# aleph-zero-foundation/sha2-on-cq-halo2

Hardware: AMD Instinct MI355X
Metric: sha256_cq_create_proof_k18: MSM Mscalar/s over proof-generation wall-clock (ms_per_step) (higher is better)
Workload: dtype u256-montgomery

## Files before the change

sha2_on_cq_halo2_amd/csrc/capi.hip:

```cpp
#include "ctx.hpp"
#include "comm.hpp"
#include "msm.hpp"
#include "poly.hpp"
#include <cstring>

using namespace cq;

const NttTables* cq_ctx::tables_for(uint32_t log_n, const Fr& omega, int* rc) {
  for (auto& t : ntt_cache)
    if (t->log_n == log_n && t->omega == omega) return t.get();
  if (ntt_cache.size() >= 16) {
    hipStreamSynchronize(stream);
    ntt_cache.erase(ntt_cache.begin());
  }
  auto t = std::make_unique<NttTables>();
  if (t->build(log_n, omega, stream) != 0) {
    *rc = fail(CQ_ERR_HIP, "building NTT twiddle tables failed");
    return nullptr;
  }
  ntt_cache.push_back(std::move(t));
  return ntt_cache.back().get();
}

extern "C" {

const char* cq_version(void) { return "cq_halo2_amd 0.1 (gfx950)"; }

int cq_ctx_create(int device, void* hip_stream, cq_ctx** out) {
  if (!out) return CQ_ERR_ARG;
  int count = 0;
  if (hipGetDeviceCount(&count) != hipSuccess || count <= 0 || device < 0 || device >= count)
    return CQ_ERR_NO_DEVICE;
  if (hipSetDevice(device) != hipSuccess) return CQ_ERR_HIP;
  cq_ctx* c = new cq_ctx();
  c->device = device;
  if (hip_stream) {
    c->stream = (hipStream_t)hip_stream;
  } else {
    if (hipStreamCreateWithFlags(&c->stream, hipStreamNonBlocking) != hipSuccess) {
      delete c;
      return CQ_ERR_HIP;
    }
    c->own_stream = true;
  }
  *out = c;
  return CQ_OK;
}

void cq_ctx_destroy(cq_ctx* c) {
  if (!c) return;
  hipSetDevice(c->device);
  for (cq_ctx* lane : c->lanes) cq_ctx_destroy(lane);
  c->lanes.clear();
  hipStreamSynchronize(c->stream);
  if (c->aux_stream) hipStreamSynchronize(c->aux_stream);
  c->ntt_cache.clear();
  cq::comm_rccl_destroy(c);
  for (const cq::GrowBuf& b : c->scratch)
    if (b.ptr) hipFree(b.ptr);
  for (const cq::GrowBuf* b : {&c->pinned, &c->pinned_msm, &c->pinned_small, &c->pinned_comm})
    if (b->ptr) hipHostFree(b->ptr);
  if (c->comm_event) hipEventDestroy(c->comm_event);
  for (auto& g : c->graphs) hipGraphExecDestroy(g.exec);
  if (c->prof_entries) hipHostFree(c->prof_entries);
  if (c->copy_done) hipEventDestroy(c->copy_done);
  if (c->copy_stream) hipStreamDestroy(c->copy_stream);
  if (c->msm_tail_event) hipEventDestroy(c->msm_tail_event);
  if (c->aux_done) hipEventDestroy(c->aux_done);
  if (c->aux_stream) hipStreamDestroy(c->aux_stream);
  if (c->fb_table) hipFree(c->fb_table);
  for (auto& t : c->msm_tables) hipFree(t.table);
  if (c->own_stream) hipStreamDestroy(c->stream);
  delete c;
}

const char* cq_last_error(const cq_ctx* c) { return c ? c->err.c_str() : "null context"; }

int cq_rccl_unique_id(uint8_t id[CQ_RCCL_UNIQUE_ID_BYTES]) {
  if (!id) return CQ_ERR_ARG;
  return cq::comm_rccl_unique_id(id);
}
int cq_ctx_comm_init_rccl(cq_ctx* c, uint32_t rank, uint32_t world, const uint8_t id[CQ_RCCL_UNIQUE_ID_BYTES]) {
  if (!c || !id || world == 0 || rank >= world) return CQ_ERR_ARG;
  CQ_HIP(c, hipSetDevice(c->device));
  return cq::comm_rccl_init(c, rank, world, id);
}
int cq_ctx_comm_selftest(cq_ctx* c) {
  if (!c) return CQ_ERR_ARG;
  CQ_HIP(c, hipSetDevice(c->device));
  return cq::comm_rccl_selftest(c);
}
int cq_ctx_comm_destroy(cq_ctx* c) {
  if (!c) return CQ_ERR_ARG;
  cq::comm_rccl_destroy(c);
  return CQ_OK;
}

int cq_ctx_set_hip_graphs(cq_ctx* c, int on) {
  if (!c) return CQ_ERR_ARG;
  c->graphs_on = on ? 1 : 0;
  return CQ_OK;
}

int cq_ctx_sync(cq_ctx* c) {
  if (!c) return CQ_ERR_ARG;
  CQ_HIP(c, hipStreamSynchronize(c->stream));
  return CQ_OK;
}

void* cq_ctx_stream(cq_ctx* c) { return c ? (void*)c->stream : nullptr; }

int cq_dev_alloc(cq_ctx* c, size_t bytes, void** dptr) {
  if (!c || !dptr) return CQ_ERR_ARG;
  CQ_HIP(c, hipSetDevice(c->device));
  CQ_HIP(c, hipMalloc(dptr, bytes ? bytes : 1));
  return CQ_OK;
}
int cq_dev_free(cq_ctx* c, void* dptr) {
  if (!c) return CQ_ERR_ARG;
  if (!dptr) return CQ_OK;
  CQ_HIP(c, hipStreamSynchronize(c->stream));
  msm_unregister_tables(c, dptr);
  CQ_HIP(c, hipFree(dptr));
  return CQ_OK;
}
int cq_dev_upload(cq_ctx* c, void* dst, const void* src, size_t bytes) {
  if (!c || (!dst && bytes) || (!src && bytes)) return CQ_ERR_ARG;
  if (!bytes) return CQ_OK;
  CQ_HIP(c, hipMemcpyAsync(dst, src, bytes, hipMemcpyHostToDevice, c->stream));
  CQ_HIP(c, hipStreamSynchronize(c->stream));
  return CQ_OK;
}
int cq_dev_download(cq_ctx* c, void* dst, const void* src, size_t bytes) {
  if (!c || (!dst && bytes) || (!src && bytes)) return CQ_ERR_ARG;
  if (!bytes) return CQ_OK;
  CQ_HIP(c, hipMemcpyAsync(dst, src, bytes, hipMemcpyDeviceToHost, c->stream));
  CQ_HIP(c, hipStreamSynchronize(c->stream));
  return CQ_OK;
}
int cq_dev_memset(cq_ctx* c, void* dptr, int value, size_t bytes) {
  if (!c || (!dptr && bytes)) return CQ_ERR_ARG;
  if (!bytes) return CQ_OK;
  CQ_HIP(c, hipMemsetAsync(dptr, value, bytes, c->stream));
  return CQ_OK;
}

int cq_profile_enable(cq_ctx* c, int on) {
  if (!c) return CQ_ERR_ARG;
  if (on && !c->prof_entries) {
    hipError_t e = hipHostMalloc((void**)&c->prof_entries, cq_ctx::PROF_COUNTERS * sizeof(uint32_t), hipHostMallocDefault);
    if (e != hipSuccess) return c->hip_fail(e, "hipHostMalloc(profile counters)");
  }
  c->prof_on = on != 0;
  return CQ_OK;
}

int cq_profile_read(cq_ctx* c, int id, double* total_ms, uint64_t* calls) {
  if (!c || !total_ms || !calls) return CQ_ERR_ARG;
  CQ_HIP(c, hipStreamSynchronize(c->stream));
  double tot = 0;
  uint64_t n = 0;
  if (id == CQ_PROF_MSM_ENTRIES) {
    for (size_t i = 0; i < c->prof_entries_n; i++) n += c->prof_entries[i];
    c->prof_entries_n = 0;
    *total_ms = 0;
    *calls = n;
    return CQ_OK;
  }
  std::vector<cq_ctx::ProfSpan> keep;
  for (auto& sp : c->prof_spans) {
    if (sp.id != id) {
      keep.push_back(sp);
      continue;
    }
    float ms = 0;
    if (hipEventElapsedTime(&ms, sp.a, sp.b) == hipSuccess) {
      tot += ms;
      n++;
    }
    hipEventDestroy(sp.a);
    hipEventDestroy(sp.b);
  }
  c->prof_spans.swap(keep);
  *total_ms = tot;
  *calls = n;
  return CQ_OK;
}

static int fft_dev(cq_ctx* c, const Fr* in, Fr* out, uint32_t log_n, const Fr& omega) {
  return domain_fft(c, in, out, log_n, omega, 1, (size_t)1 << log_n, (size_t)1 << log_n);
}

int cq_best_fft_dev(cq_ctx* c, const uint64_t* in_dev, uint64_t* out_dev, uint32_t log_n,
                    const uint64_t omega[4]) {
  if (!c || !in_dev || !out_dev || !omega || log_n > FR_S) return CQ_ERR_ARG;
  CQ_HIP(c, hipSetDevice(c->device));
  return fft_dev(c, (const Fr*)in_dev, (Fr*)out_dev, log_n, Fr::from_limbs64(omega));
}

int cq_best_fft(cq_ctx* c, uint64_t* a, uint32_t log_n, const uint64_t omega[4]) {
  if (!c || !a || !omega || log_n > FR_S) return CQ_ERR_ARG;
  CQ_HIP(c, hipSetDevice(c->device));
  const size_t bytes = ((size_t)1 << log_n) * sizeof(Fr);
  void *din, *dout;
  int rc;
  if ((rc = c->ensure_scratch(Scratch::EntryA, bytes, &din)) != CQ_OK) return rc;
  if ((rc = c->ensure_scratch(Scratch::EntryB, bytes, &dout)) != CQ_OK) return rc;
  CQ_HIP(c, hipMemcpyAsync(din, a, bytes, hipMemcpyHostToDevice, c->stream));
  if ((rc = fft_dev(c, (const Fr*)din, (Fr*)dout, log_n, Fr::from_limbs64(omega))) != CQ_OK) return rc;
  CQ_HIP(c, hipMemcpyAsync(a, dout, bytes, hipMemcpyDeviceToHost, c->stream));
  CQ_HIP(c, hipStreamSynchronize(c->stream));
  return CQ_OK;
}

}
```

sha2_on_cq_halo2_amd/csrc/capi_msm.hip:

```cpp
#include <algorithm>
#include <cstdlib>
#include <cstring>
#include <string>
#include <vector>
#include "ctx.hpp"
#include "msm.hpp"
#include "g1fft.hpp"
#include "setup.hpp"
#include "cq.hpp"
#include "serde.hpp"
#include "msm_g2.hpp"

using namespace cq;

uint32_t msm_table_window_bits(size_t n) {
  if (const char* e = getenv("CQ_TABLE_C")) {
    const long v = atol(e);
    if (v >= (long)MSM_TABLE_C_MIN && v <= (long)MSM_TABLE_C_MAX) return (uint32_t)v;
  }
  return n >= ((size_t)1 << 20) ? 17u : MSM_TABLE_C;
}

static uint32_t pick_c(cq_ctx* c, uint32_t n) {
  if (c->msm_c) return c->msm_c;
  return msm_window_bits(n);
}

int msm_multi_begin(cq_ctx* c, const Fr* const* scalars, const G1Affine* const* bases, const size_t* lens, size_t count,
                    MsmPending& pend) {
  pend.launches.clear();
  pend.count = count;
  for (size_t j = 0; j < count; j++)
    if (lens[j] > 0x7fffffffull) return c->fail(CQ_ERR_ARG, "msm: len too large");
  uint32_t want_c = 0;
  {
    size_t longest = 0;
    for (size_t j = 0; j < count; j++)
      if (lens[j] > longest)
        if (const cq_ctx::MsmTable* t = c->find_msm_table(bases[j], lens[j])) { longest = lens[j]; want_c = t->c; }
  }
  size_t done = 0, slots = 0;
  while (done < count) {
    MsmPending::Launch ln;
    ln.first = done;
    if (lens[done] == 0) {
      ln.batch = 1;
      ln.empty = true;
      pend.launches.push_back(ln);
      done++;
      continue;
    }
    const cq_ctx::MsmTable* t0 = c->find_msm_table(bases[done], lens[done], nullptr, want_c);
    const bool pre = t0 != nullptr;
    uint32_t nmax = (uint32_t)lens[done];
    uint32_t batch = 1;
    while (done + batch < count && batch < MSM_MAX_BATCH) {
      const size_t l = lens[done + batch];
      if (l == 0) break;
      const cq_ctx::MsmTable* t = c->find_msm_table(bases[done + batch], l, nullptr, want_c);
      if ((t != nullptr) != pre) break;
      if (pre && t->c != t0->c) break;
      if (!pre && l != lens[done]) break;
      nmax = std::max(nmax, (uint32_t)l);
      batch++;
    }
    ln.short_path = !pre && !c->msm_c && nmax <= MSM_SHORT_MAX;
    const uint32_t cb = pre ? t0->c : ln.short_path ? MSM_SHORT_C : pick_c(c, nmax);
    while (batch > 1 && MsmLayout(nmax, cb, batch, pre).total > ((size_t)32 << 30)) batch = (batch + 1) / 2;
    ln.batch = batch;
    ln.pre = pre;
    ln.c = cb;
    ln.nmax = nmax;
    MsmLayout L(nmax, cb, batch, pre);
    ln.W = L.W;
    ln.Wb = L.Wb;
    ln.M = L.M;
    ln.cols = L.cols;
    ln.slot = slots;
    slots += (size_t)MSM_SET_POINTS * batch * L.Wb;
    pend.launches.push_back(ln);
    done += batch;
  }
  void *wsums = nullptr, *host = nullptr;
  int rc;
  if (slots) {
    if ((rc = c->ensure_scratch(Scratch::MsmSums, slots * sizeof(G1Jac), &wsums)) != CQ_OK) return rc;
    if ((rc = c->ensure_pinned_msm(slots * sizeof(G1Jac), &host)) != CQ_OK) return rc;
  }
  pend.host = host;
  pend.slots = slots;
  for (auto& ln : pend.launches) {
    if (ln.empty) continue;
    if (ln.short_path) {
      void* ws;
      if ((rc = c->ensure_scratch(Scratch::MsmWork, msm_short_workspace(ln.nmax, ln.batch), &ws)) != CQ_OK) return rc;
      if (msm_short_run(c, scalars + ln.first, bases + ln.first, ln.nmax, ln.batch, ws, (G1Jac*)wsums + ln.slot) != 0)
        return c->fail(CQ_ERR_HIP, "msm launch failed");
      continue;
    }
    MsmLayout L(ln.nmax, ln.c, ln.batch, ln.pre);
    std::vector<const G1Affine*> bp(ln.batch);
    std::vector<size_t> strides(ln.batch, 0);
    for (uint32_t j = 0; j < ln.batch; j++) {
      size_t toff = 0;
      const cq_ctx::MsmTable* t = ln.pre ? c->find_msm_table(bases[ln.first + j], lens[ln.first + j], &toff, ln.c) : nullptr;
      bp[j] = ln.pre ? (const G1Affine*)t->table + toff : bases[ln.first + j];
      strides[j] = ln.pre ? t->n : 0;
    }
    void* ws;
    if ((rc = c->ensure_scratch(Scratch::MsmWork, L.total, &ws)) != CQ_OK) return rc;
    int r = msm_run(c, scalars + ln.first, bp.data(), lens + ln.first, ln.nmax, ln.c, ln.batch, ln.pre, strides.data(), ws,
                    (G1Jac*)wsums + ln.slot);
    if (r != 0) return c->fail(CQ_ERR_HIP, "msm launch failed");
  }
  if (slots)
    CQ_HIP(c, hipMemcpyAsync(host, wsums, slots * sizeof(G1Jac), hipMemcpyDeviceToHost, c->stream));
  return CQ_OK;
}

int msm_multi_end(cq_ctx* c, MsmPending& pend, uint64_t* out_jac) {
  if (int wrc = c->wait(c->stream, "msm: waiting for the launch")) return wrc;
  struct Item { const MsmPending::Launch* ln; uint32_t j; };
  std::vector<Item> items;
  size_t sets = 0;
  for (auto& ln : pend.launches)
    for (uint32_t j = 0; j < ln.batch; j++) {
      items.push_back({&ln, j});
      if (!ln.empty) sets += ln.Wb;
    }
  const G1Jac* host = (const G1Jac*)pend.host;
  auto fold = [&](size_t i) {
    const MsmPending::Launch& ln = *items[i].ln;
    const uint32_t j = items[i].j;
    uint64_t* o = out_jac + (ln.first + j) * 12;
    if (ln.empty) {
      memset(o, 0, 12 * sizeof(uint64_t));
      return;
    }
    const G1Jac* res = host + ln.slot;
    G1Jac r = ln.pre ? msm_fold_sets(res + (size_t)MSM_SET_POINTS * j * ln.Wb, ln.Wb, ln.M, ln.cols)
                     : msm_fold_windows(res + (size_t)MSM_SET_POINTS * j * ln.W, ln.W, ln.c, ln.cols);
    r.x.to_limbs64(o);
    r.y.to_limbs64(o + 4);
    r.z.to_limbs64(o + 8);
  };
  if (sets > 6) {
    c->pool().parallel_for(items.size(), fold);
  } else {
    for (size_t i = 0; i < items.size(); i++) fold(i);
  }
  return CQ_OK;
}

int cq_msm_multi_v(cq_ctx* c, const Fr* const* scalars, const G1Affine* const* bases, const size_t* lens, size_t count,
                   uint64_t* out_jac) {
  MsmPending pend;
  int rc = msm_multi_begin(c, scalars, bases, lens, count, pend);
  if (rc != CQ_OK) return rc;
  return msm_multi_end(c, pend, out_jac);
}

int cq_msm_multi(cq_ctx* c, const Fr* const* scalars, const G1Affine* const* bases, size_t len, size_t count,
                 uint64_t* out_jac) {
  std::vector<size_t> lens(count, len);
  return cq_msm_multi_v(c, scalars, bases, lens.data(), count, out_jac);
}

void msm_unregister_tables(cq_ctx* c, const void* bases) {
  for (size_t i = 0; i < c->msm_tables.size();) {
    if (c->msm_tables[i].bases == bases) {
      hipFree(c->msm_tables[i].table);
      c->msm_tables.erase(c->msm_tables.begin() + i);
    } else {
      i++;
    }
  }
}

void msm_release_table(cq_ctx* c, const void* bases, size_t n, uint32_t c_bits) {
  for (size_t i = 0; i < c->msm_tables.size(); i++) {
    cq_ctx::MsmTable& t = c->msm_tables[i];
    if (t.bases != bases || t.n != n || t.c != c_bits) continue;
    if (--t.refs == 0) {
      hipFree(t.table);
      c->msm_tables.erase(c->msm_tables.begin() + i);
    }
    return;
  }
}

int msm_register_tables(cq_ctx* c, const G1Affine* bases, size_t n, uint32_t want_c, bool* held) {
  if (held) *held = false;
  if (!bases || n == 0 || n > (1u << 26)) return CQ_OK;
  const uint32_t cb = want_c ? want_c : (c->msm_table_c ? c->msm_table_c : msm_table_window_bits(n));
  for (auto& t : c->msm_tables)
    if (t.bases == bases && t.n == n && t.c == cb) {
      t.refs++;
      if (held) *held = true;
      return CQ_OK;
    }
  {
    size_t off = 0;
    const cq_ctx::MsmTable* t = c->find_msm_table(bases, n, &off, cb);
    if (t && (t->c == cb || !want_c)) return CQ_OK;
  }
  const uint32_t W = (255 + cb - 1) / cb;
  void* table = nullptr;
  if (hipMalloc(&table, (size_t)W * n * sizeof(G1Affine)) != hipSuccess) {
    (void)hipGetLastError();
    return CQ_OK;
  }
  if (msm_precompute_tables(c, bases, (uint32_t)n, cb, (G1Affine*)table) != 0) {
    hipFree(table);
    return c->fail(CQ_ERR_HIP, "msm precompute failed");
  }
  c->msm_tables.push_back({bases, n, cb, table, 1});
  if (held) *held = true;
  return CQ_OK;
}

static int msm_batch(cq_ctx* c, const Fr* const* scalars, const G1Affine* bases, size_t len, size_t count,
                     uint64_t* out_jac) {
  std::vector<const G1Affine*> bp(count, bases);
  return cq_msm_multi(c, scalars, bp.data(), len, count, out_jac);
}

namespace {
struct ParamsGuard {
  cq_params* p;
  explicit ParamsGuard(cq_params* p_) : p(p_) {}
  ~ParamsGuard() {
    if (p) cq_params_destroy(p);
  }
  cq_params* release() {
    cq_params* q = p;
    p = nullptr;
    return q;
  }
};
cq_params* params_new(cq_ctx* c, uint32_t k) {
  cq_params* p = new cq_params();
  p->ctx = c;
  p->k = k;
  p->n = (size_t)1 << k;
  p->g = nullptr;
  p->g_lagrange = nullptr;
  return p;
}
}

extern "C" {

int cq_msm_precompute_dev(cq_ctx* c, const uint64_t* bases_dev, size_t n) {
  if (!c || !bases_dev) return CQ_ERR_ARG;
  CQ_HIP(c, hipSetDevice(c->device));
  return msm_register_tables(c, (const G1Affine*)bases_dev, n);
}

int cq_msm_forget_dev(cq_ctx* c, const uint64_t* bases_dev) {
  if (!c || !bases_dev) return CQ_ERR_ARG;
  CQ_HIP(c, hipStreamSynchronize(c->stream));
  msm_unregister_tables(c, bases_dev);
  return CQ_OK;
}

int cq_msm_set_precompute(cq_ctx* c, int on) {
  if (!c) return CQ_ERR_ARG;
  c->msm_precompute = on != 0;
  return CQ_OK;
}

int cq_msm_set_table_window(cq_ctx* c, uint32_t bits) {
  if (!c || (bits != 0 && (bits < MSM_TABLE_C_MIN || bits > MSM_TABLE_C_MAX))) return CQ_ERR_ARG;
  c->msm_table_c = bits;
  return CQ_OK;
}

int cq_msm_table_width_dev(cq_ctx* c, const uint64_t* bases_dev, size_t n, uint32_t preferred_bits, uint32_t* bits) {
  if (!c || !bases_dev || !bits) return CQ_ERR_ARG;
  const cq_ctx::MsmTable* t = c->find_msm_table(bases_dev, n, nullptr, preferred_bits);
  *bits = t ? t->c : 0;
  return CQ_OK;
}

int cq_msm_bucket_sums_dev(cq_ctx* c, const uint64_t* const* bases_dev, size_t arrays, int packed, const uint32_t* index_dev, size_t n,
                           size_t buckets, uint64_t* out_dev) {
  if (!c || !bases_dev || !index_dev || !out_dev || !arrays || arrays > MSM_MAX_BATCH || !n || n > ((size_t)1 << 26) || !buckets ||
      buckets > ((size_t)1 << (MSM_TABLE_C - 1)))
    return CQ_ERR_ARG;
  CQ_HIP(c, hipSetDevice(c->device));
  void* conv = nullptr;
  int rc;
  if (!packed && (rc = c->ensure_scratch(Scratch::EntryB, arrays * n * sizeof(G1Affine), &conv)) != CQ_OK) return rc;
  std::vector<const uint32_t*> idx(arrays, index_dev);
  std::vector<const G1Affine*> bs(arrays);
  for (size_t a = 0; a < arrays; a++) {
    if (!bases_dev[a]) return CQ_ERR_ARG;
    bs[a] = (const G1Affine*)bases_dev[a];
    if (!packed) {
      G1Affine* dst = (G1Affine*)conv + a * n;
      if (msm_bases29(c, bs[a], (uint32_t)n, dst) != 0) return c->fail(CQ_ERR_HIP, "bucket sums: bases");
      bs[a] = dst;
// ... 440 lines not shown
```

sha2_on_cq_halo2_amd/csrc/ctx.hpp:

```cpp
#pragma once
#include <hip/hip_runtime.h>
#include <cstdlib>
#include <memory>
#include <string>
#include <vector>
#include "../../include/cq_halo2.h"
#include "field.hpp"
#include "ntt.hpp"
#include "hostpool.hpp"

namespace cq {
int comm_rccl_wait(cq_ctx* c, hipStream_t stream, const char* what);

enum class Scratch {
  Ntt,
  EntryA,
  EntryB,
  MsmWork,
  MsmSums,
  PolyTmp,
  ProverArena,
  ProverStage,
  HostAdvice,
  NttAux,
  CommGather,
  Check,
  Count
};

struct GrowBuf {
  void* ptr = nullptr;
  size_t bytes = 0;
};
}

struct cq_ctx {
  int device = 0;
  hipStream_t stream = nullptr;
  bool own_stream = false;
  std::string err;
  std::vector<std::unique_ptr<cq::NttTables>> ntt_cache;
  cq::GrowBuf scratch[(int)cq::Scratch::Count];
  cq::GrowBuf pinned;
  uint32_t msm_c = 0;
  uint32_t msm_table_c = 0;
  bool msm_precompute = true;
  void* fb_table = nullptr;
  struct MsmTable { const void* bases; size_t n; uint32_t c; void* table; uint32_t refs; };
  std::vector<MsmTable> msm_tables;
  cq_ctx* parent = nullptr;
  std::vector<cq_ctx*> lanes;
  const MsmTable* find_msm_table(const void* bases, size_t len, size_t* offset = nullptr, uint32_t want_c = 0) const {
    if (parent) return parent->find_msm_table(bases, len, offset, want_c);
    const MsmTable* any = nullptr;
    size_t any_off = 0;
    for (auto& t : msm_tables) {
      const char* b0 = (const char*)t.bases;
      const char* b = (const char*)bases;
      if (b < b0 || b >= b0 + t.n * 64) continue;
      const size_t off = (size_t)(b - b0) / 64;
      if ((size_t)(b - b0) % 64 || off + len > t.n) continue;
      if (!any) { any = &t; any_off = off; }
      if (want_c == 0 || t.c == want_c) {
        if (offset) *offset = off;
        return &t;
      }
    }
    if (any && offset) *offset = any_off;
    return any;
  }
  struct ProfSpan { int id; hipEvent_t a, b; };
  bool prof_on = false;
  std::vector<ProfSpan> prof_spans;
  static constexpr size_t PROF_COUNTERS = 4096;
  uint32_t* prof_entries = nullptr;
  size_t prof_entries_n = 0;
  hipEvent_t prof_begin(int id) {
    if (!prof_on) return nullptr;
    ProfSpan sp;
    sp.id = id;
    hipEventCreate(&sp.a);
    hipEventCreate(&sp.b);
    hipEventRecord(sp.a, stream);
    prof_spans.push_back(sp);
    return sp.b;
  }
  void prof_end(hipEvent_t b) {
    if (b) hipEventRecord(b, stream);
  }

  int wait(hipStream_t s, const char* what = "stream wait") {
    if (rccl_comm) return cq::comm_rccl_wait(this, s, what);
    const hipError_t e = hipStreamSynchronize(s);
    return e == hipSuccess ? CQ_OK : hip_fail(e, what);
  }

  int fail(int code, const std::string& msg) {
    err = msg;
    return code;
  }
  int hip_fail(hipError_t e, const char* what) {
    err = std::string(what) + ": " + hipGetErrorString(e);
    return CQ_ERR_HIP;
  }
  int grow(cq::GrowBuf& b, size_t bytes, size_t min_bytes, bool host, void** out) {
    if (b.bytes < bytes) {
      if (b.ptr) {
        hipStreamSynchronize(stream);
        host ? hipHostFree(b.ptr) : hipFree(b.ptr);
        b = {};
      }
      const size_t want = bytes < min_bytes ? min_bytes : bytes;
      const hipError_t e = host ? hipHostMalloc(&b.ptr, want, hipHostMallocDefault) : hipMalloc(&b.ptr, want);
      if (e != hipSuccess) return hip_fail(e, host ? "hipHostMalloc" : "hipMalloc(scratch)");
      b.bytes = want;
    }
    *out = b.ptr;
    return CQ_OK;
  }
  int ensure_scratch(cq::Scratch s, size_t bytes, void** out) { return grow(scratch[(int)s], bytes, 1u << 20, false, out); }
  int ensure_pinned(size_t bytes, void** out) { return grow(pinned, bytes, 0, true, out); }
  hipStream_t copy_stream = nullptr;
  hipEvent_t copy_done = nullptr;
  int ensure_copy_stream() {
    if (copy_stream) return CQ_OK;
    hipError_t e = hipStreamCreateWithFlags(&copy_stream, hipStreamNonBlocking);
    if (e != hipSuccess) return hip_fail(e, "hipStreamCreate(copy)");
    e = hipEventCreateWithFlags(&copy_done, hipEventDisableTiming);
    if (e != hipSuccess) return hip_fail(e, "hipEventCreate(copy)");
    return CQ_OK;
  }
  hipStream_t aux_stream = nullptr;
  hipEvent_t msm_tail_event = nullptr, aux_done = nullptr;
  uint64_t msm_tail_seq = 0;
  bool aux_pending = false;
  int ensure_aux_stream() {
    if (aux_stream) return CQ_OK;
    int least = 0, greatest = 0;
    (void)hipDeviceGetStreamPriorityRange(&least, &greatest);
    hipError_t e = hipStreamCreateWithPriority(&aux_stream, hipStreamNonBlocking, least);
    if (e != hipSuccess) return hip_fail(e, "hipStreamCreate(aux)");
    e = hipEventCreateWithFlags(&msm_tail_event, hipEventDisableTiming);
    if (e == hipSuccess) e = hipEventCreateWithFlags(&aux_done, hipEventDisableTiming);
    if (e != hipSuccess) return hip_fail(e, "hipEventCreate(aux)");
    return CQ_OK;
  }
  struct GraphEntry { std::vector<uint64_t> sig; int segment; hipGraphExec_t exec; };
  std::vector<GraphEntry> graphs;
  int graphs_on = -1;
  template <class F>
  int run_graph(const std::vector<uint64_t>& sig, int segment, F&& enqueue) {
    if (graphs_on < 0) {
      const char* e = getenv("CQ_HIP_GRAPH");
      graphs_on = (e && e[0] == '1') ? 1 : 0;
    }
    if (!graphs_on) return enqueue();
    for (auto& g : graphs)
      if (g.segment == segment && g.sig == sig) {
        if (hipGraphLaunch(g.exec, stream) == hipSuccess) return 0;
        graphs_on = 0;
        (void)hipGetLastError();
        return enqueue();
      }
    if (hipStreamBeginCapture(stream, hipStreamCaptureModeThreadLocal) != hipSuccess) {
      graphs_on = 0;
      (void)hipGetLastError();
      return enqueue();
    }
    const int rc = enqueue();
    hipGraph_t graph = nullptr;
    const hipError_t ec = hipStreamEndCapture(stream, &graph);
    hipGraphExec_t exec = nullptr;
    if (rc != 0 || ec != hipSuccess || !graph || hipGraphInstantiate(&exec, graph, nullptr, nullptr, 0) != hipSuccess) {
      if (graph) hipGraphDestroy(graph);
      graphs_on = 0;
      (void)hipGetLastError();
      return rc != 0 ? rc : enqueue();
    }
    hipGraphDestroy(graph);
    if (graphs.size() >= 64) {
      for (auto& g : graphs) hipGraphExecDestroy(g.exec);
      graphs.clear();
    }
    graphs.push_back({sig, segment, exec});
    if (hipGraphLaunch(exec, stream) == hipSuccess) return 0;
    graphs_on = 0;
    (void)hipGetLastError();
    return enqueue();
  }
  std::unique_ptr<cq::HostPool> pool_;
  cq::HostPool& pool() {
    if (parent) return parent->pool();
    if (!pool_) {
      unsigned hw = std::thread::hardware_concurrency();
      unsigned w = hw > 3 ? (hw - 2 < 12 ? hw - 2 : 12) : 0;
      if (const char* e = getenv("CQ_HOST_THREADS")) w = (unsigned)atoi(e);
      pool_.reset(new cq::HostPool(w));
    }
    return *pool_;
  }
  cq::GrowBuf pinned_small;
  static constexpr size_t PINNED_SMALL_BYTES = 16384;
  int ensure_pinned_small(void** out) { return grow(pinned_small, PINNED_SMALL_BYTES, PINNED_SMALL_BYTES, true, out); }
  void* rccl_comm = nullptr;
  uint32_t rccl_rank = 0, rccl_world = 1;
  bool rccl_aborted = false;
  hipEvent_t comm_event = nullptr;
  cq::GrowBuf pinned_comm;
  int ensure_pinned_comm(size_t bytes, void** out) { return grow(pinned_comm, bytes, 65536, true, out); }
  cq::GrowBuf pinned_msm;
  int ensure_pinned_msm(size_t bytes, void** out) { return grow(pinned_msm, bytes, 65536, true, out); }
  const cq::NttTables* tables_for(uint32_t log_n, const cq::Fr& omega, int* rc);
};

#define CQ_HIP(ctx, call)                                   \
  do {                                                      \
    hipError_t _e = (call);                                 \
    if (_e != hipSuccess) return (ctx)->hip_fail(_e, #call); \
  } while (0)
```

sha2_on_cq_halo2_amd/csrc/hostpool.hpp:

```cpp
#pragma once
#include <atomic>
#include <condition_variable>
#include <deque>
#include <functional>
#include <memory>
#include <mutex>
#include <thread>
#include <vector>

namespace cq {

class HostPool {
 public:
  struct Job {
    std::function<void(size_t)> fn;
    size_t count = 0;
    std::atomic<size_t> next{0}, done{0};
  };
  using Ticket = std::shared_ptr<Job>;

  explicit HostPool(unsigned workers) {
    for (unsigned i = 0; i < workers; i++) {
      try {
        threads_.emplace_back([this]() { run(); });
      } catch (...) {
        break;
      }
    }
  }
  ~HostPool() {
    {
      std::lock_guard<std::mutex> lk(mu_);
      stop_ = true;
    }
    cv_.notify_all();
    for (auto& t : threads_) t.join();
  }
  HostPool(const HostPool&) = delete;
  HostPool& operator=(const HostPool&) = delete;

  Ticket submit(size_t count, std::function<void(size_t)> fn) {
    Ticket j = std::make_shared<Job>();
    j->fn = std::move(fn);
    j->count = count;
    if (count && !threads_.empty()) {
      {
        std::lock_guard<std::mutex> lk(mu_);
        queue_.push_back(j);
      }
      cv_.notify_all();
    }
    return j;
  }
  void wait(const Ticket& j) {
    if (!j) return;
    work_on(*j);
    std::unique_lock<std::mutex> lk(mu_);
    done_cv_.wait(lk, [&]() { return j->done.load() >= j->count; });
  }
  void parallel_for(size_t count, std::function<void(size_t)> fn) { wait(submit(count, std::move(fn))); }

 private:
  void work_on(Job& j) {
    for (;;) {
      const size_t i = j.next.fetch_add(1);
      if (i >= j.count) return;
      j.fn(i);
      if (j.done.fetch_add(1) + 1 == j.count) {
        std::lock_guard<std::mutex> lk(mu_);
        done_cv_.notify_all();
      }
    }
  }
  void run() {
    for (;;) {
      Ticket j;
      {
        std::unique_lock<std::mutex> lk(mu_);
        cv_.wait(lk, [&]() { return stop_ || !queue_.empty(); });
        if (stop_) return;
        j = queue_.front();
        if (j->next.load() >= j->count) {
          queue_.pop_front();
          continue;
        }
      }
      work_on(*j);
    }
  }
  std::vector<std::thread> threads_;
  std::deque<Ticket> queue_;
  std::mutex mu_;
  std::condition_variable cv_, done_cv_;
  bool stop_ = false;
};

}
```

sha2_on_cq_halo2_amd/csrc/msm.hpp:

```cpp
#pragma once
#include <hip/hip_runtime.h>
#include <vector>
#include "curve.hpp"

struct cq_ctx;

namespace cq {

constexpr uint32_t MSM_ACC_THREADS = 128;

#ifndef CQ_MSM_S1
#define CQ_MSM_S1 24
#endif
constexpr uint32_t MSM_S1 = CQ_MSM_S1;
#ifndef CQ_MSM_S1_BIG
#define CQ_MSM_S1_BIG 32
#endif
#ifndef CQ_MSM_S1_BIG_LOAD
#define CQ_MSM_S1_BIG_LOAD 512
#endif
constexpr uint32_t MSM_S1_BIG = CQ_MSM_S1_BIG;
constexpr uint32_t MSM_S1_BIG_LOAD = CQ_MSM_S1_BIG_LOAD;
#ifndef CQ_MSM_PARTIALS_TARGET
#define CQ_MSM_PARTIALS_TARGET 48
#endif
constexpr uint32_t MSM_PARTIALS_TARGET = CQ_MSM_PARTIALS_TARGET;
static_assert(MSM_S1_BIG >= MSM_S1, "the workspace is sized for MSM_S1");
#ifndef CQ_MSM_SMALL_LANES
#define CQ_MSM_SMALL_LANES 65536
#endif
constexpr uint32_t MSM_S1_MIN = 4;
constexpr uint64_t MSM_SMALL_LANES = CQ_MSM_SMALL_LANES;
__host__ __device__ inline uint32_t msm_small_launch_s1(uint64_t entry_bound) {
  if (entry_bound >= (uint64_t)MSM_S1 * MSM_SMALL_LANES) return MSM_S1;
  const uint64_t s = entry_bound / MSM_SMALL_LANES;
  return (uint32_t)(s < MSM_S1_MIN ? MSM_S1_MIN : s);
}
constexpr uint64_t MSM_SMALL_PARTIALS = 3 * MSM_SMALL_LANES;
constexpr uint32_t MSM_S2 = 64;
constexpr uint32_t MSM_SHORT = 64;
constexpr uint32_t MSM_SHORT_MIN = 16;
#ifndef CQ_MSM_WAVE_BUDGET
#define CQ_MSM_WAVE_BUDGET 4096
#endif
constexpr uint32_t MSM_WAVE_BUDGET = CQ_MSM_WAVE_BUDGET;
constexpr uint32_t MSM_COMBINE_WAVE_BLOCKS = 2048;
constexpr uint32_t MSM_MAX_BATCH = 32;
constexpr uint32_t MSM_SET_POINTS = 15;

constexpr uint32_t MSM_SHORT_C = 8, MSM_SHORT_W = 32;
constexpr uint32_t MSM_SHORT_LIMIT = 1u << 14;
#ifndef CQ_MSM_SHORT_MAX
#define CQ_MSM_SHORT_MAX 16384
#endif
constexpr uint32_t MSM_SHORT_MAX = CQ_MSM_SHORT_MAX;
static_assert(MSM_SHORT_MAX <= MSM_SHORT_LIMIT && MSM_SHORT_MAX >= 4097, "the cut-over covers N + 1 = 4097 and fits the kernel");

struct MsmPtrs {
  const void* p[MSM_MAX_BATCH];
};
struct MsmStrides {
  uint64_t s[MSM_MAX_BATCH];
};

struct MsmLayout {
  uint32_t n, c, batch, W, Wb, M, B, Bt, levels, nseq, nblk, rows, cols, npart, nfinal, shift1;
  bool pre, part_sort, mid;
  uint64_t tmax[8];
  size_t off_ptrs, off_ranks, off_poff, off_poff2, off_counts, off_cursor, off_psize, off_psize2, off_buckets, off_ticket, zero_end, off_blocksums,
      off_off, off_tk, off_sorted, off_part[2], off_pairs, total;
  MsmLayout(uint32_t n_, uint32_t c_, uint32_t batch_, bool pre_ = false);
};

uint32_t msm_window_bits(uint32_t n);
int msm_run(cq_ctx* ctx, const Fr* const* scalars, const G1Affine* const* bases, const size_t* lens, uint32_t n, uint32_t c,
            uint32_t batch, bool pre, const size_t* table_strides, void* workspace, G1Jac* window_sums_dev,
            G1Affine* raw_out = nullptr, uint32_t raw_count = 0, const uint32_t* const* index = nullptr);
size_t msm_short_workspace(uint32_t n, uint32_t batch);
int msm_short_run(cq_ctx* ctx, const Fr* const* scalars, const G1Affine* const* bases, uint32_t n, uint32_t batch, void* workspace,
                  G1Jac* window_sums_dev);
int msm_bucket_sums(cq_ctx* ctx, const uint32_t* const* index, const G1Affine* const* bases29, uint32_t n, uint32_t batch, uint32_t count,
                    G1Affine* out);
int msm_bases29(cq_ctx* ctx, const G1Affine* bases, uint32_t n, G1Affine* out);
bool msm_bucket_sums_fit(uint32_t n, uint32_t batch);
int msm_precompute_tables(cq_ctx* ctx, const G1Affine* bases, uint32_t n, uint32_t c, G1Affine* table);
G1Jac msm_set_value(const G1Jac* planes, uint32_t cols);
G1Jac msm_fold_windows(const G1Jac* pairs, uint32_t W, uint32_t c, uint32_t cols);
G1Jac msm_fold_sets(const G1Jac* pairs, uint32_t Wb, uint32_t M, uint32_t cols);

}

int cq_msm_multi(cq_ctx* c, const cq::Fr* const* scalars, const cq::G1Affine* const* bases, size_t len, size_t count,
                 uint64_t* out_jac);
int cq_msm_multi_v(cq_ctx* c, const cq::Fr* const* scalars, const cq::G1Affine* const* bases, const size_t* lens, size_t count,
                   uint64_t* out_jac);
struct MsmPending {
  struct Launch {
    size_t first = 0, slot = 0;
    uint32_t batch = 0, c = 0, nmax = 0, W = 0, Wb = 0, M = 0, cols = 0;
    bool pre = false, empty = false;
    bool short_path = false;
  };
  std::vector<Launch> launches;
  void* host = nullptr;
  size_t slots = 0, count = 0;
};
int msm_multi_begin(cq_ctx* c, const cq::Fr* const* scalars, const cq::G1Affine* const* bases, const size_t* lens, size_t count,
                    MsmPending& pend);
int msm_multi_end(cq_ctx* c, MsmPending& pend, uint64_t* out_jac);
constexpr uint32_t MSM_TABLE_C = 15, MSM_TABLE_C_MIN = 8, MSM_TABLE_C_MAX = 20;
uint32_t msm_table_window_bits(size_t n);

int msm_register_tables(cq_ctx* c, const cq::G1Affine* bases, size_t n, uint32_t want_c = 0, bool* held = nullptr);
void msm_release_table(cq_ctx* c, const void* bases, size_t n, uint32_t c_bits);
void msm_unregister_tables(cq_ctx* c, const void* bases);
```

sha2_on_cq_halo2_amd/csrc/prover.hip:

```cpp
#include <algorithm>
#include <array>
#include <atomic>
#include <chrono>
#include <cstdio>
#include <cstdlib>
#include <cstring>
#include <thread>
#include <vector>
#include "blake2b.hpp"
#include "comm.hpp"
#include "cq.hpp"
#include "ctx.hpp"
#include "msm.hpp"
#include "plonk.hpp"
#include "prover.hpp"
#include "glv.hpp"
#include "xoshiro.hpp"

using namespace cq;

namespace {

struct Transcript {
  Blake2b st;
  std::vector<uint8_t> proof;
  Transcript() { st.init(64, "Halo2-Transcript"); }
  void common_scalar(const Fr& s) {
    const uint8_t tag = 2;
    st.update(&tag, 1);
    U256 c = s.to_canonical();
    st.update((const uint8_t*)c.l, 32);
  }
  bool common_point(const G1Affine& p) {
    if (p.is_identity()) return false;
    const uint8_t tag = 1;
    st.update(&tag, 1);
    U256 x = p.x.to_canonical(), y = p.y.to_canonical();
    st.update((const uint8_t*)x.l, 32);
    st.update((const uint8_t*)y.l, 32);
    return true;
  }
  bool write_point(const G1Affine& p) {
    if (!common_point(p)) return false;
    U256 x = p.x.to_canonical(), y = p.y.to_canonical();
    uint8_t b[32];
    memcpy(b, x.l, 32);
    b[31] |= (uint8_t)((y.l[0] & 1) << 7);
    proof.insert(proof.end(), b, b + 32);
    return true;
  }
  void write_scalar(const Fr& s) {
    common_scalar(s);
    U256 c = s.to_canonical();
    const uint8_t* b = (const uint8_t*)c.l;
    proof.insert(proof.end(), b, b + 32);
  }
  Fr squeeze() {
    const uint8_t tag = 0;
    st.update(&tag, 1);
    uint8_t out[64];
    st.finalize_clone(out);
    uint64_t w[8];
    memcpy(w, out, 64);
    return Fr::from_u512(w);
  }
};

void batch_normalize(const std::vector<G1Jac>& in, std::vector<G1Affine>& out) {
  out.resize(in.size());
  std::vector<Fq> pref(in.size());
  Fq acc = Fq::one();
  for (size_t i = 0; i < in.size(); i++) {
    pref[i] = acc;
    if (!in[i].is_identity()) acc = acc * in[i].z;
  }
  acc = acc.inv();
  for (size_t i = in.size(); i-- > 0;) {
    if (in[i].is_identity()) {
      out[i] = G1Affine::identity();
      continue;
    }
    Fq zi = pref[i] * acc;
    acc = acc * in[i].z;
    Fq zi2 = zi.sqr();
    out[i] = {in[i].x * zi2, in[i].y * zi2 * zi};
  }
}

G1Jac jac_from_limbs(const uint64_t* l) {
  return {Fq::from_limbs64(l), Fq::from_limbs64(l + 4), Fq::from_limbs64(l + 8)};
}

struct Rng {
  cq_rng_next_u64 next;
  void* state;
  cq_rng_fill_fn bulk = nullptr;
  HostPool* pool = nullptr;
  void words(uint64_t* w8) {
    for (int i = 0; i < 8; i++) w8[i] = next(state);
  }
  Fr fr() {
    uint64_t w[8];
    words(w);
    return Fr::from_u512(w);
  }
  void fill(uint64_t* dst, size_t count) {
    if (bulk) {
      bulk(state, dst, count);
    } else if (next == cq_xoshiro256ss_next_u64) {
      xoshiro_fill((uint64_t*)state, dst, count, 8, pool);
    } else if (next == cq_buffer_rng_next_u64) {
      cq_buffer_rng* b = (cq_buffer_rng*)state;
      const size_t avail = b->pos < b->len ? b->len - b->pos : 0, take = std::min(avail, count);
      memcpy(dst, b->words + b->pos, take * sizeof(uint64_t));
      memset(dst + take, 0, (count - take) * sizeof(uint64_t));
      b->pos += take;
      b->overrun += count - take;
    } else {
      for (size_t i = 0; i < count; i++) dst[i] = next(state);
    }
  }
};

struct Commit {
  const cq_pk* pk;
  MsmPending pend;
  size_t count = 0;
  int begin(const cq_pk* pk_, const std::vector<const Fr*>& scalars, const std::vector<const G1Affine*>& bases,
            const std::vector<size_t>& lens) {
    pk = pk_;
    count = scalars.size();
    if (!pk->sharded()) return msm_multi_begin(pk->ctx, scalars.data(), bases.data(), lens.data(), count, pend);
    std::vector<const Fr*> sc(count);
    std::vector<const G1Affine*> bs(count);
    std::vector<size_t> ln(count);
    for (size_t j = 0; j < count; j++) {
      size_t lo, hi;
      shard_range(lens[j], pk->shard_rank, pk->shard_world, lo, hi);
      sc[j] = scalars[j] + lo;
      bs[j] = bases[j] + lo;
      ln[j] = hi - lo;
    }
    return msm_multi_begin(pk->ctx, sc.data(), bs.data(), ln.data(), count, pend);
  }
  int end(std::vector<G1Affine>& out) {
    cq_ctx* c = pk->ctx;
    std::vector<uint64_t> jac(count * 12);
    static const bool trace_host = getenv("CQ_TRACE_HOST") != nullptr;
    const auto t0 = std::chrono::steady_clock::now();
    if (trace_host) hipStreamSynchronize(c->stream);
    const auto t1 = std::chrono::steady_clock::now();
    int rc = msm_multi_end(c, pend, jac.data());
    if (rc != CQ_OK) return rc;
    const auto t2 = std::chrono::steady_clock::now();
    struct Report {
      bool on; std::chrono::steady_clock::time_point a, b, c_;
      ~Report() {
        if (on) fprintf(stderr, "[cq host]   commit end: wait %.1f us, fold %.1f us, exchange + normalise %.1f us\n",
                        std::chrono::duration<double, std::micro>(b - a).count(), std::chrono::duration<double, std::micro>(c_ - b).count(),
                        std::chrono::duration<double, std::micro>(std::chrono::steady_clock::now() - c_).count());
      }
    } report{trace_host, t0, t1, t2};
    std::vector<G1Jac> j(count);
    if (pk->sharded()) {
      std::vector<uint64_t> all((size_t)pk->shard_world * count * 12);
      int arc = shard_allgather_host(pk, jac.data(), all.data(), count * 12 * sizeof(uint64_t));
      if (arc != CQ_OK) return arc;
      for (size_t i = 0; i < count; i++) {
        G1Jac acc = G1Jac::identity();
        for (uint32_t r = 0; r < pk->shard_world; r++) acc = jac_add(acc, jac_from_limbs(all.data() + ((size_t)r * count + i) * 12));
        j[i] = acc;
      }
    } else {
      for (size_t i = 0; i < count; i++) j[i] = jac_from_limbs(jac.data() + 12 * i);
    }
    batch_normalize(j, out);
    return CQ_OK;
  }
};

int shard_any(const cq_pk* pk, bool flag, bool& out) {
  out = flag;
  if (!pk->sharded()) return CQ_OK;
  const uint64_t mine = flag ? 1 : 0;
  std::vector<uint64_t> all(pk->shard_world, 0);
  int arc = shard_allgather_host(pk, &mine, all.data(), sizeof(uint64_t));
  if (arc != CQ_OK) return arc;
  for (uint64_t v : all) out = out || v != 0;
  return CQ_OK;
}

struct AuxFork {
  cq_ctx* c;
  hipStream_t main = nullptr;
  bool active = false;
  explicit AuxFork(cq_ctx* c_) : c(c_) {}
  int begin(uint64_t seq_before) {
    if (c->msm_tail_seq == seq_before) CQ_HIP(c, hipEventRecord(c->msm_tail_event, c->stream));
    CQ_HIP(c, hipStreamWaitEvent(c->aux_stream, c->msm_tail_event, 0));
    main = c->stream;
    c->stream = c->aux_stream;
    active = true;
    return CQ_OK;
  }
  int end() {
    if (!active) return CQ_OK;
    restore();
    c->aux_pending = true;
    CQ_HIP(c, hipEventRecord(c->aux_done, c->aux_stream));
    return CQ_OK;
  }
  void restore() {
    c->stream = main;
    active = false;
  }
  ~AuxFork() {
    if (active) {
      restore();
      hipStreamSynchronize(c->aux_stream);
    }
  }
};
static int join_aux(cq_ctx* c) {
  if (!c->aux_pending) return CQ_OK;
  c->aux_pending = false;
  CQ_HIP(c, hipStreamWaitEvent(c->stream, c->aux_done, 0));
  return CQ_OK;
}

int commit_batch_v(const cq_pk* pk, const std::vector<const Fr*>& scalars, const std::vector<const G1Affine*>& bases,
                   const std::vector<size_t>& lens, std::vector<G1Affine>& out) {
  Commit cm;
  int rc = cm.begin(pk, scalars, bases, lens);
  if (rc != CQ_OK) return rc;
  return cm.end(out);
}

int commit_batch(const cq_pk* pk, const std::vector<const Fr*>& scalars, const std::vector<const G1Affine*>& bases, size_t len,
                 std::vector<G1Affine>& out) {
  std::vector<size_t> lens(scalars.size(), len);
  return commit_batch_v(pk, scalars, bases, lens, out);
}

}

#define CQ_TRY(x)               \
  do {                          \
    int _rc = (x);              \
    if (_rc != CQ_OK) return _rc; \
  } while (0)

namespace cq {

namespace {

struct Arena {
  Fr* base;
  size_t used = 0;
  Fr* take(size_t elems) {
    Fr* p = base ? base + used : nullptr;
    used += elems;
    return p;
  }
};
struct Buffers {
  Fr *adv, *adv_coeff, *inst_lag, *inst_coeff, *f_lag, *f_coeff, *bpoly, *random_poly, *z, *mv, *cosets, *adv_cosets, *inst_cosets,
      *z_cosets, *lk_inputs, *plk, *plk_cosets, *h_ext, *h_coeff, *gwc_batch, *gwc_wit, *shplonk, *t_comp, *den, *a_val, *m_fr, *a_scaled;
  Fr* challenges;
  Fr* b_values;
  G1Affine* b_sums;
  Fr *tails, *gather;
  uint64_t* rng_dev;
  uint32_t *m_counts, *err_dev;
};

std::vector<int32_t> opening_rotations(const cq_pk* pk) {
  std::vector<int32_t> rots{0};
  auto seen = [&](int32_t r) {
    if (std::find(rots.begin(), rots.end(), r) == rots.end()) rots.push_back(r);
  };
  for (auto& q : pk->advice_queries) seen(q.second);
  for (auto& q : pk->fixed_queries) seen(q.second);
  if (pk->perm_sets() || !pk->legacy.empty()) seen(1);
  if (!pk->legacy.empty()) seen(-1);
  if (pk->perm_sets() > 1) seen(-(int32_t)(pk->bf + 1));
  return rots;
}

bool early_advice_polys(const cq_pk* pk) {
  return !pk->general() && pk->perm_sets() == 0 && pk->num_phases == 1 && pk->num_advice > 0 && !pk->lookups.empty();
}

void carve(const cq_pk* pk, Arena& ar, Buffers& b) {
  const size_t n = (size_t)1 << pk->k, ext = pk->domain->ext();
  const size_t L = pk->lookups.size(), A = pk->num_advice, I = pk->num_instance, S = pk->perm_sets();
  const size_t N = pk->table_cfg ? pk->table_cfg->N : 0;
  const bool general = pk->general();
  size_t wsum = 0;
  for (auto& lk : pk->lookups) wsum += lk.cols.size();
  const size_t npts = opening_rotations(pk).size();
  b.adv = ar.take(A * n);
  b.adv_coeff = ar.take(early_advice_polys(pk) ? A * n : 0);
  b.inst_lag = ar.take(I * n);
  b.inst_coeff = ar.take(I * n);
  b.f_lag = ar.take(L * n);
  b.f_coeff = ar.take(L * n);
  b.bpoly = ar.take(L * n);
  b.den = ar.take(L * N + 8);
  b.random_poly = ar.take(n);
  b.z = ar.take(S * n);
  b.mv = ar.take(S * n);
  b.cosets = ar.take(2 * L * ext);
  b.adv_cosets = ar.take(general ? A * ext : 0);
  b.inst_cosets = ar.take(general ? I * ext : 0);
  b.z_cosets = ar.take(S * ext);
// ... 1276 lines not shown
```

Baseline: 1316.

## Overlap host-side MSM window folding with remaining GPU launches via early per-launch copies

For multi-launch MSM batches, every non-empty launch except the last is marked early. Its window sums are copied device-to-host on a separate copy stream right after it is launched, and host pool workers wait on per-launch events and fold those results while later launches still run. msm_multi_end then folds only the remaining launches and joins the early work. The aim is to hide host fold and transfer latency behind GPU compute, at the cost of extra events, thread-pool contention, and more complex lifetime handling.

```diff
diff --git a/sha2_on_cq_halo2_amd/csrc/capi.hip b/sha2_on_cq_halo2_amd/csrc/capi.hip
--- a/sha2_on_cq_halo2_amd/csrc/capi.hip
+++ b/sha2_on_cq_halo2_amd/csrc/capi.hip
@@ -52,8 +52,11 @@
   hipSetDevice(c->device);
   for (cq_ctx* lane : c->lanes) cq_ctx_destroy(lane);
   c->lanes.clear();
+  if (c->msm_early) c->msm_early->join();
+  c->msm_early.reset();
   hipStreamSynchronize(c->stream);
   if (c->aux_stream) hipStreamSynchronize(c->aux_stream);
+  if (c->copy_stream) hipStreamSynchronize(c->copy_stream);
   c->ntt_cache.clear();
   cq::comm_rccl_destroy(c);
   for (const cq::GrowBuf& b : c->scratch)
@@ -63,6 +66,7 @@
   if (c->comm_event) hipEventDestroy(c->comm_event);
   for (auto& g : c->graphs) hipGraphExecDestroy(g.exec);
   if (c->prof_entries) hipHostFree(c->prof_entries);
+  for (hipEvent_t ev : c->msm_early_events) hipEventDestroy(ev);
   if (c->copy_done) hipEventDestroy(c->copy_done);
   if (c->copy_stream) hipStreamDestroy(c->copy_stream);
   if (c->msm_tail_event) hipEventDestroy(c->msm_tail_event);
diff --git a/sha2_on_cq_halo2_amd/csrc/capi_msm.hip b/sha2_on_cq_halo2_amd/csrc/capi_msm.hip
--- a/sha2_on_cq_halo2_amd/csrc/capi_msm.hip
+++ b/sha2_on_cq_halo2_amd/csrc/capi_msm.hip
@@ -1,4 +1,5 @@
 #include <algorithm>
+#include <chrono>
 #include <cstdlib>
 #include <cstring>
 #include <string>
@@ -26,8 +27,14 @@
   return msm_window_bits(n);
 }
 
-int msm_multi_begin(cq_ctx* c, const Fr* const* scalars, const G1Affine* const* bases, const size_t* lens, size_t count,
-                    MsmPending& pend) {
+static G1Jac fold_one(const G1Jac* host, const MsmPending::Launch& ln, uint32_t j) {
+  const G1Jac* res = host + ln.slot;
+  return ln.pre ? msm_fold_sets(res + (size_t)MSM_SET_POINTS * j * ln.Wb, ln.Wb, ln.M, ln.cols)
+                : msm_fold_windows(res + (size_t)MSM_SET_POINTS * j * ln.W, ln.W, ln.c, ln.cols);
+}
+
+static int msm_multi_begin_impl(cq_ctx* c, const Fr* const* scalars, const G1Affine* const* bases, const size_t* lens, size_t count,
+                                MsmPending& pend, hipStream_t* early_copy_on) {
   pend.launches.clear();
   pend.count = count;
   for (size_t j = 0; j < count; j++)
@@ -81,6 +88,18 @@
     pend.launches.push_back(ln);
     done += batch;
   }
+  size_t n_early = 0, early_items = 0;
+  if (!c->rccl_comm && c->pool().workers() > 0) {
+    MsmPending::Launch* last = nullptr;
+    for (auto& ln : pend.launches)
+      if (!ln.empty) last = &ln;
+    for (auto& ln : pend.launches)
+      if (!ln.empty && &ln != last) {
+        ln.early = true;
+        n_early++;
+        early_items += ln.batch;
+      }
+  }
   void *wsums = nullptr, *host = nullptr;
   int rc;
   if (slots) {
@@ -89,6 +108,17 @@
   }
   pend.host = host;
   pend.slots = slots;
+  std::shared_ptr<MsmEarlyFold> ef;
+  hipStream_t copy_on = c->stream;
+  if (n_early) {
+    if ((rc = c->ensure_msm_early_events(n_early)) != CQ_OK) return rc;
+    if (c->ensure_copy_stream() == CQ_OK) copy_on = c->copy_stream;
+    ef = std::make_shared<MsmEarlyFold>();
+    ef->pool = &c->pool();
+    ef->host = (const G1Jac*)host;
+    ef->items.reserve(early_items);
+  }
+  size_t early_seen = 0, copied_to = 0;
   for (auto& ln : pend.launches) {
     if (ln.empty) continue;
     if (ln.short_path) {
@@ -96,26 +126,78 @@
       if ((rc = c->ensure_scratch(Scratch::MsmWork, msm_short_workspace(ln.nmax, ln.batch), &ws)) != CQ_OK) return rc;
       if (msm_short_run(c, scalars + ln.first, bases + ln.first, ln.nmax, ln.batch, ws, (G1Jac*)wsums + ln.slot) != 0)
         return c->fail(CQ_ERR_HIP, "msm launch failed");
-      continue;
-    }
-    MsmLayout L(ln.nmax, ln.c, ln.batch, ln.pre);
-    std::vector<const G1Affine*> bp(ln.batch);
-    std::vector<size_t> strides(ln.batch, 0);
+    } else {
+      MsmLayout L(ln.nmax, ln.c, ln.batch, ln.pre);
+      std::vector<const G1Affine*> bp(ln.batch);
+      std::vector<size_t> strides(ln.batch, 0);
+      for (uint32_t j = 0; j < ln.batch; j++) {
+        size_t toff = 0;
+        const cq_ctx::MsmTable* t = ln.pre ? c->find_msm_table(bases[ln.first + j], lens[ln.first + j], &toff, ln.c) : nullptr;
+        bp[j] = ln.pre ? (const G1Affine*)t->table + toff : bases[ln.first + j];
+        strides[j] = ln.pre ? t->n : 0;
+      }
+      void* ws;
+      if ((rc = c->ensure_scratch(Scratch::MsmWork, L.total, &ws)) != CQ_OK) return rc;
+      int r = msm_run(c, scalars + ln.first, bp.data(), lens + ln.first, ln.nmax, ln.c, ln.batch, ln.pre, strides.data(), ws,
+                      (G1Jac*)wsums + ln.slot);
+      if (r != 0) return c->fail(CQ_ERR_HIP, "msm launch failed");
+    }
+    if (!ln.early) continue;
+    const hipEvent_t launched = c->msm_early_events[2 * early_seen], copied = c->msm_early_events[2 * early_seen + 1];
+    early_seen++;
+    const size_t points = (size_t)MSM_SET_POINTS * ln.batch * ln.Wb;
+    if (copy_on != c->stream) {
+      CQ_HIP(c, hipEventRecord(launched, c->stream));
+      CQ_HIP(c, hipStreamWaitEvent(copy_on, launched, 0));
+    }
+    *early_copy_on = copy_on;
+    CQ_HIP(c, hipMemcpyAsync((G1Jac*)host + ln.slot, (const G1Jac*)wsums + ln.slot, points * sizeof(G1Jac), hipMemcpyDeviceToHost, copy_on));
+    CQ_HIP(c, hipEventRecord(copied, copy_on));
+    copied_to = ln.slot + points;
     for (uint32_t j = 0; j < ln.batch; j++) {
-      size_t toff = 0;
-      const cq_ctx::MsmTable* t = ln.pre ? c->find_msm_table(bases[ln.first + j], lens[ln.first + j], &toff, ln.c) : nullptr;
-      bp[j] = ln.pre ? (const G1Affine*)t->table + toff : bases[ln.first + j];
-      strides[j] = ln.pre ? t->n : 0;
-    }
-    void* ws;
-    if ((rc = c->ensure_scratch(Scratch::MsmWork, L.total, &ws)) != CQ_OK) return rc;
-    int r = msm_run(c, scalars + ln.first, bp.data(), lens + ln.first, ln.nmax, ln.c, ln.batch, ln.pre, strides.data(), ws,
-                    (G1Jac*)wsums + ln.slot);
-    if (r != 0) return c->fail(CQ_ERR_HIP, "msm launch failed");
-  }
-  if (slots)
-    CQ_HIP(c, hipMemcpyAsync(host, wsums, slots * sizeof(G1Jac), hipMemcpyDeviceToHost, c->stream));
-  return CQ_OK;
+      MsmEarlyFold::Item it;
+      it.ln = ln;
+      it.j = j;
+      it.copied = copied;
+      ef->items.push_back(it);
+    }
+  }
+  if (slots > copied_to)
+    CQ_HIP(c, hipMemcpyAsync((G1Jac*)host + copied_to, (const G1Jac*)wsums + copied_to, (slots - copied_to) * sizeof(G1Jac), hipMemcpyDeviceToHost,
+                             c->stream));
+  if (ef) {
+    ef->out.resize(ef->items.size());
+    ef->t_done.resize(ef->items.size());
+    ef->t_submit = std::chrono::steady_clock::now();
+    std::fill(ef->t_done.begin(), ef->t_done.end(), ef->t_submit);
+    MsmEarlyFold* st = ef.get();
+    pend.early = ef;
+    c->msm_early = ef;
+    ef->ticket = ef->pool->submit(st->items.size(), [st](size_t i) {
+      const MsmEarlyFold::Item& it = st->items[i];
+      const hipError_t e = hipEventSynchronize(it.copied);
+      if (e != hipSuccess) {
+        (void)hipGetLastError();
+        st->hip_err.store((int)e);
+      } else {
+        st->out[i] = fold_one(st->host, it.ln, it.j);
+      }
+      st->t_done[i] = std::chrono::steady_clock::now();
+    });
+  }
+  return CQ_OK;
+}
+
+int msm_multi_begin(cq_ctx* c, const Fr* const* scalars, const G1Affine* const* bases, const size_t* lens, size_t count,
+                    MsmPending& pend) {
+  if (pend.early) pend.early->join();
+  pend.early.reset();
+  if (c->msm_early) c->msm_early->join();
+  c->msm_early.reset();
+  hipStream_t early_copy_on = nullptr;
+  const int rc = msm_multi_begin_impl(c, scalars, bases, lens, count, pend, &early_copy_on);
+  if (rc != CQ_OK && early_copy_on && !pend.early) (void)hipStreamSynchronize(early_copy_on);
+  return rc;
 }
 
 int msm_multi_end(cq_ctx* c, MsmPending& pend, uint64_t* out_jac) {
@@ -123,31 +205,39 @@
   struct Item { const MsmPending::Launch* ln; uint32_t j; };
   std::vector<Item> items;
   size_t sets = 0;
-  for (auto& ln : pend.launches)
+  for (auto& ln : pend.launches) {
+    if (ln.early) continue;
     for (uint32_t j = 0; j < ln.batch; j++) {
       items.push_back({&ln, j});
       if (!ln.empty) sets += ln.Wb;
     }
+  }
   const G1Jac* host = (const G1Jac*)pend.host;
+  auto put = [&](const G1Jac& r, size_t index) {
+    uint64_t* o = out_jac + index * 12;
+    r.x.to_limbs64(o);
+    r.y.to_limbs64(o + 4);
+    r.z.to_limbs64(o + 8);
+  };
   auto fold = [&](size_t i) {
     const MsmPending::Launch& ln = *items[i].ln;
     const uint32_t j = items[i].j;
-    uint64_t* o = out_jac + (ln.first + j) * 12;
     if (ln.empty) {
-      memset(o, 0, 12 * sizeof(uint64_t));
+      memset(out_jac + (ln.first + j) * 12, 0, 12 * sizeof(uint64_t));
       return;
     }
-    const G1Jac* res = host + ln.slot;
-    G1Jac r = ln.pre ? msm_fold_sets(res + (size_t)MSM_SET_POINTS * j * ln.Wb, ln.Wb, ln.M, ln.cols)
-                     : msm_fold_windows(res + (size_t)MSM_SET_POINTS * j * ln.W, ln.W, ln.c, ln.cols);
-    r.x.to_limbs64(o);
-    r.y.to_limbs64(o + 4);
-    r.z.to_limbs64(o + 8);
+    put(fold_one(host, ln, j), ln.first + j);
   };
   if (sets > 6) {
     c->pool().parallel_for(items.size(), fold);
   } else {
     for (size_t i = 0; i < items.size(); i++) fold(i);
+  }
+  if (MsmEarlyFold* ef = pend.early.get()) {
+    ef->end_waited = ef->ticket && ef->ticket->done.load() < ef->ticket->count;
+    ef->join();
+    if (const int e = ef->hip_err.load()) return c->hip_fail((hipError_t)e, "msm: waiting for an early launch's results");
+    for (size_t i = 0; i < ef->items.size(); i++) put(ef->out[i], ef->items[i].ln.first + ef->items[i].j);
   }
   return CQ_OK;
 }
diff --git a/sha2_on_cq_halo2_amd/csrc/ctx.hpp b/sha2_on_cq_halo2_amd/csrc/ctx.hpp
--- a/sha2_on_cq_halo2_amd/csrc/ctx.hpp
+++ b/sha2_on_cq_halo2_amd/csrc/ctx.hpp
@@ -33,6 +33,8 @@
   size_t bytes = 0;
 };
 }
+
+struct MsmEarlyFold;
 
 struct cq_ctx {
   int device = 0;
@@ -210,6 +212,17 @@
   int ensure_pinned_comm(size_t bytes, void** out) { return grow(pinned_comm, bytes, 65536, true, out); }
   cq::GrowBuf pinned_msm;
   int ensure_pinned_msm(size_t bytes, void** out) { return grow(pinned_msm, bytes, 65536, true, out); }
+  std::vector<hipEvent_t> msm_early_events;
+  std::shared_ptr<MsmEarlyFold> msm_early;
+  int ensure_msm_early_events(size_t launches) {
+    while (msm_early_events.size() < 2 * launches) {
+      hipEvent_t ev = nullptr;
+      const hipError_t e = hipEventCreateWithFlags(&ev, hipEventDisableTiming);
+      if (e != hipSuccess) return hip_fail(e, "hipEventCreate(msm early fold)");
+      msm_early_events.push_back(ev);
+    }
+    return CQ_OK;
+  }
   const cq::NttTables* tables_for(uint32_t log_n, const cq::Fr& omega, int* rc);
 };
 
diff --git a/sha2_on_cq_halo2_amd/csrc/hostpool.hpp b/sha2_on_cq_halo2_amd/csrc/hostpool.hpp
--- a/sha2_on_cq_halo2_amd/csrc/hostpool.hpp
+++ b/sha2_on_cq_halo2_amd/csrc/hostpool.hpp
@@ -59,6 +59,7 @@
     done_cv_.wait(lk, [&]() { return j->done.load() >= j->count; });
   }
   void parallel_for(size_t count, std::function<void(size_t)> fn) { wait(submit(count, std::move(fn))); }
+  size_t workers() const { return threads_.size(); }
 
  private:
   void work_on(Job& j) {
diff --git a/sha2_on_cq_halo2_amd/csrc/msm.hpp b/sha2_on_cq_halo2_amd/csrc/msm.hpp
--- a/sha2_on_cq_halo2_amd/csrc/msm.hpp
+++ b/sha2_on_cq_halo2_amd/csrc/msm.hpp
@@ -1,7 +1,11 @@
 #pragma once
 #include <hip/hip_runtime.h>
+#include <atomic>
+#include <chrono>
+#include <memory>
 #include <vector>
 #include "curve.hpp"
+#include "hostpool.hpp"
 
 struct cq_ctx;
 
@@ -94,17 +98,53 @@
                  uint64_t* out_jac);
 int cq_msm_multi_v(cq_ctx* c, const cq::Fr* const* scalars, const cq::G1Affine* const* bases, const size_t* lens, size_t count,
                    uint64_t* out_jac);
+struct MsmEarlyFold;
 struct MsmPending {
   struct Launch {
     size_t first = 0, slot = 0;
     uint32_t batch = 0, c = 0, nmax = 0, W = 0, Wb = 0, M = 0, cols = 0;
     bool pre = false, empty = false;
     bool short_path = false;
+    bool early = false;
   };
   std::vector<Launch> launches;
   void* host = nullptr;
   size_t slots = 0, count = 0;
+  std::shared_ptr<MsmEarlyFold> early;
+  MsmPending() = default;
+  MsmPending(const MsmPending&) = delete;
+  MsmPending& operator=(const MsmPending&) = delete;
+  ~MsmPending();
 };
+struct MsmEarlyFold {
+  struct Item {
+    MsmPending::Launch ln;
+    uint32_t j = 0;
+    hipEvent_t copied = nullptr;
+  };
+  cq::HostPool* pool = nullptr;
+  cq::HostPool::Ticket ticket;
+  std::vector<Item> items;
+  std::vector<cq::G1Jac> out;
+  std::vector<std::chrono::steady_clock::time_point> t_done;
+  std::chrono::steady_clock::time_point t_submit;
+  const cq::G1Jac* host = nullptr;
+  std::atomic<int> hip_err{0};
+  bool end_waited = false;
+  void join() {
+    if (ticket) pool->wait(ticket);
+    ticket.reset();
+  }
+  double span_us() const {
+    auto last = t_submit;
+    for (auto& t : t_done) last = t > last ? t : last;
+    return std::chrono::duration<double, std::micro>(last - t_submit).count();
+  }
+  ~MsmEarlyFold() { join(); }
+};
+inline MsmPending::~MsmPending() {
+  if (early) early->join();
+}
 int msm_multi_begin(cq_ctx* c, const cq::Fr* const* scalars, const cq::G1Affine* const* bases, const size_t* lens, size_t count,
                     MsmPending& pend);
 int msm_multi_end(cq_ctx* c, MsmPending& pend, uint64_t* out_jac);
diff --git a/sha2_on_cq_halo2_amd/csrc/prover.hip b/sha2_on_cq_halo2_amd/csrc/prover.hip
--- a/sha2_on_cq_halo2_amd/csrc/prover.hip
+++ b/sha2_on_cq_halo2_amd/csrc/prover.hip
@@ -155,12 +155,16 @@
     const auto t2 = std::chrono::steady_clock::now();
     struct Report {
       bool on; std::chrono::steady_clock::time_point a, b, c_;
+      const MsmEarlyFold* early;
       ~Report() {
-        if (on) fprintf(stderr, "[cq host]   commit end: wait %.1f us, fold %.1f us, exchange + normalise %.1f us\n",
-                        std::chrono::duration<double, std::micro>(b - a).count(), std::chrono::duration<double, std::micro>(c_ - b).count(),
-                        std::chrono::duration<double, std::micro>(std::chrono::steady_clock::now() - c_).count());
-      }
-    } report{trace_host, t0, t1, t2};
+        if (!on) return;
+        fprintf(stderr, "[cq host]   commit end: wait %.1f us, fold %.1f us, exchange + normalise %.1f us",
+                std::chrono::duration<double, std::micro>(b - a).count(), std::chrono::duration<double, std::micro>(c_ - b).count(),
+                std::chrono::duration<double, std::micro>(std::chrono::steady_clock::now() - c_).count());
+        if (early) fprintf(stderr, "; early fold: %zu items, %.1f us, end waited: %s", early->items.size(), early->span_us(), early->end_waited ? "yes" : "no");
+        fprintf(stderr, "\n");
+      }
+    } report{trace_host, t0, t1, t2, pend.early.get()};
     std::vector<G1Jac> j(count);
     if (pk->sharded()) {
       std::vector<uint64_t> all((size_t)pk->shard_world * count * 12);
```

Measured after the change: 1355, median of 6. 1.03x the previous value.
